# keshaviyengar/gym-ctr-reach

Hardware: AMD Instinct MI355X
Metric: env-steps/sec at 65 536 parallel 3-tube envs; tip-pos L2 vs CPU ref (higher is better)
Workload: dtype f64; 1 GPU; configs[2]: 65536 envs/GPU, 3-tube torsionally-compliant CTR, scipy-RK45 (rtol 1e-3, atol 1e-6) fp64, system 0, n_substeps 10, tol 0.020, max 150 steps, auto-reset; obs_dtype=float32, integrator=rk45_scipy, model=compliant, envs_per_gpu=65536, global_envs=65536, parallelism=env-shard x1, launch=one HIP graph per refill period (2 steps + the refill), replayed

## Files before the change

gym-ctr-reach_amd/csrc/ctr_kernels.hip:

```cpp
#include <hip/hip_runtime.h>
#include <stdint.h>
#include <stdio.h>
#include <string.h>

#include <algorithm>

#include "ctr_device.hpp"
#include "ctr_reach_amd.h"

using namespace ctr;

namespace {

constexpr int BLOCK = 256;

thread_local char g_err[512] = "";

int fail(int code, const char *msg)
{
    snprintf(g_err, sizeof g_err, "%s", msg);
    return code;
}

int hip_check(const char *what)
// ... 462 lines not shown
    #pragma unroll
    for (int i = 27; i < 32; ++i) d[i] = 0u;
    uint4 *v = reinterpret_cast<uint4 *>(sl);
    #pragma unroll
    for (int k = 0; k < 8; ++k) v[k] = make_uint4(d[4 * k], d[4 * k + 1], d[4 * k + 2], d[4 * k + 3]);
}

template <bool ALL = false>
__device__ __forceinline__ void pool_prefetch(const KCfg &kc, const ctr_batch_t &b, int64_t e, int32_t autoreset,
                                              PoolPre &pp, int32_t t, uint32_t epoch)
{
    const int P = b.pool_depth;
    if (!autoreset || P <= 0 || (!ALL && t + 1 < kc.c.max_steps)) return;
    const uint32_t r = epoch + 1;
    pool_load(b.pool + ((int64_t)(r % (uint32_t)P) * b.n + e), pp);
}

struct StepFlags {
    bool miss = false;
    bool pooled = false;
    uint32_t pooled_r = 0;
};

__device__ __forceinline__ void step_finish(const KCfg &kc, const ctr_batch_t &b, const ctr_step_out_t &o, int64_t e,
                                            int s, float q[6], double ag[3], const FkStats &st, int32_t autoreset,
                                            StepFlags &fl, const ctr_her_t *her, const float *action,
                                            PoolPre &lp, int32_t t_prev, uint32_t epoch, const double dg_prev[3],
                                            float4 &grow)
{
    const int32_t t = t_prev + 1;
    double dg[3];
    #pragma unroll
    for (int i = 0; i < 3; ++i) dg[i] = dg_prev[i];
    const double dx = ag[0] - dg[0], dy = ag[1] - dg[1], dz = ag[2] - dg[2];
    const double d = sqrt(dx * dx + dy * dy + dz * dz);
    const double tol = kc.c.tol;
    const float reward = (d > tol) ? -1.0f : 0.0f;
    const bool done = (reward == 0.0f) || (t >= kc.c.max_steps);
    const bool multi = kc.c.n_systems > 1;
    const bool f64 = kc.c.obs_f64 != 0;
    double obs[14];
    obs_lane(q, dg, ag, tol, s, multi, kc.c.egocentric != 0, obs);
    o.reward[e] = reward;
    o.done[e] = done ? 1 : 0;
    o.success[e] = (d < tol) ? 1 : 0;
    o.error[e] = (float)d;
    uint32_t stat = st.status;
    if (o.nfev) o.nfev[e] = st.nfev;
    if (o.packed || o.gather) {
        const float fl = (float)((done ? 1 : 0) | ((d < tol) ? 2 : 0) | ((reward < 0.0f) ? 4 : 0));
        const float4 row = make_float4((float)ag[0], (float)ag[1], (float)ag[2], fl);
        if (o.packed) *reinterpret_cast<float4 *>(o.packed + 4 * e) = row;
        grow = row;
    }
    if (her) {
        float obf[14];
        obs_to_f32(obs, obf);
        her_record_lane(*her, e, action, reward, done, obf, ag, tol);
    }
    int32_t t_out = t;
    if (autoreset && done) {
        if (o.terminal_obs) write_obs(o.terminal_obs, e, obs, multi, f64);
        if (o.terminal_achieved)
            #pragma unroll
            for (int i = 0; i < 3; ++i) o.terminal_achieved[3 * e + i] = ag[i];
        const uint32_t r = epoch + 1;
        const int P = b.pool_depth;
        if (P > 0 && !lp.loaded) pool_load(b.pool + ((int64_t)(r % (uint32_t)P) * b.n + e), lp);
        if (P > 0 && lp.pr == r) {
            const int s2 = clamp_sys(lp.sys, kc.c.n_systems);
            #pragma unroll
            for (int i = 0; i < 6; ++i) q[i] = lp.q0[i];
            #pragma unroll
            for (int i = 0; i < 3; ++i) {
                dg[i] = lp.dg[i];
                ag[i] = lp.ag[i];
            }
            if (b.desired_joints)
                #pragma unroll
                for (int i = 0; i < 6; ++i) b.desired_joints[6 * e + i] = lp.qd[i];
            if (b.starting_joints)
                #pragma unroll
                for (int i = 0; i < 6; ++i) b.starting_joints[6 * e + i] = q[i];
            if (b.starting_position)
                #pragma unroll
                for (int i = 0; i < 3; ++i) b.starting_position[3 * e + i] = ag[i];
            #pragma unroll
            for (int i = 0; i < 3; ++i) b.desired_goal[3 * e + i] = dg[i];
            b.system[e] = s2;
            b.epoch[e] = r;
            stat |= lp.stat;
            obs_lane(q, dg, ag, kc.c.tol, s2, multi, kc.c.egocentric != 0, obs);
            if (her) {
                float obf[14];
                obs_to_f32(obs, obf);
                her_reopen(*her, e, r, obf, ag, dg);
            }
            fl.pooled = true;
            fl.pooled_r = r;
            t_out = 0;
        } else if (autoreset == CTR_AUTORESET_POOLED) {
            stat |= CTR_STATUS_POOL_MISS;
        } else {
            fl.miss = true;
        }
    }
    b.t[e] = t_out;
    #pragma unroll
    for (int i = 0; i < 6; ++i) b.joints[6 * e + i] = q[i];
    #pragma unroll
    for (int i = 0; i < 3; ++i) b.achieved_goal[3 * e + i] = ag[i];
    write_obs(o.obs, e, obs, multi, f64);
    if (o.status) o.status[e] = stat;
}

template <int G = SEG_GROUP>
__device__ __forceinline__ void step_finish_group(const KCfg &kc, const ctr_batch_t &b, const ctr_step_out_t &o,
                                                  int64_t e, int j, bool in, int s, const float q[6], double ag[3],
                                                  const FkStats &st, int32_t autoreset, StepFlags &fl,
                                                  PoolPre &pp, float4 &grow)
{
    const int lead = (int)(threadIdx.x & 63) & ~(G - 1);
    #pragma unroll
    for (int i = 0; i < 3; ++i) ag[i] = __shfl(ag[i], lead);
    if (!in || j > 1) return;
    const int32_t t = b.t[e] + 1;
    double dg[3];
    #pragma unroll
    for (int i = 0; i < 3; ++i) dg[i] = b.desired_goal[3 * e + i];
    const double dx = ag[0] - dg[0], dy = ag[1] - dg[1], dz = ag[2] - dg[2];
    const double d = sqrt(dx * dx + dy * dy + dz * dz);
    const double tol = kc.c.tol;
    const float reward = (d > tol) ? -1.0f : 0.0f;
    const bool done = (reward == 0.0f) || (t >= kc.c.max_steps);
    const bool multi = kc.c.n_systems > 1;
    const bool f64 = kc.c.obs_f64 != 0;
// ... 50 lines not shown
            #pragma unroll
            for (int i = 0; i < 6; ++i) b.desired_joints[6 * e + i] = pp.qd[i];
        if (b.starting_joints)
            #pragma unroll
            for (int i = 0; i < 6; ++i) b.starting_joints[6 * e + i] = pp.q0[i];
        if (b.starting_position)
            #pragma unroll
            for (int i = 0; i < 3; ++i) b.starting_position[3 * e + i] = pp.ag[i];
        #pragma unroll
        for (int i = 0; i < 3; ++i) { b.desired_goal[3 * e + i] = pp.dg[i]; b.achieved_goal[3 * e + i] = pp.ag[i]; }
        #pragma unroll
        for (int i = 0; i < 6; ++i) b.joints[6 * e + i] = pp.q0[i];
        b.system[e] = so;
        b.epoch[e] = r;
        b.t[e] = 0;
        write_obs(o.obs, e, obs, multi, f64);
        fl.pooled = true;
        fl.pooled_r = r;
    }
}

__device__ __forceinline__ void step_epilogue(const ctr_batch_t &b, const ctr_step_out_t &o, int32_t autoreset,
                                              const StepFlags &fl, int64_t e, bool live, const ctr_gather_push_t *gp,
                                              bool slot_free0, float4 grow)
{
    if (autoreset) {
        if (autoreset == CTR_AUTORESET_POOLED) {
            if (blockIdx.x == 0 && threadIdx.x == 0) b.work[(b.work_parity & 1) ^ 1] = 0;
        } else {
            const int32_t one[1] = {(int32_t)e};
            wave_append(miss_counter(b), miss_items(b), b.n, fl.miss, one, 1);
        }
        if (b.pool_depth > 0) {
            const int32_t two[2] = {(int32_t)e, (int32_t)(fl.pooled_r + (uint32_t)b.pool_depth)};
            wave_append(b.refill, b.refill + 1, b.refill_cap, fl.pooled, two, 2);
        }
    }
    if (gp) {
        if (!slot_free0 && !gather_wait_slot(gp, o.gather_seq)) {
            if ((threadIdx.x & 63) == 0) atomicOr(gp->err, CTR_GATHER_E_RELEASE_TIMEOUT);
            gather_poison_lanes(gp, o.gather_seq);
        }
        if (live) gather_store_row(gp, e, grow);
        gather_rows_performed();
        if (o.gather_wait_prev && blockIdx.x == 0 && threadIdx.x < 64)
            gather_wait_prev_lane(gp, o.gather_seq - 1u);
    }
}

template <int MODE, bool HER>
__device__ __forceinline__ void step_body(const KCfg &kc, const ctr_batch_t &b, const float *__restrict__ actions,
                                          const ctr_step_out_t &o, int32_t autoreset, const HerK &hk)
{
    const ctr_her_t *her = HER ? &hk.h : nullptr;
    constexpr bool GROUP = (MODE & 6) == 6;
    constexpr int G = GROUP ? SEG_GROUP : 1;
    __shared__ SysK s_sys[CTR_MAX_SYSTEMS];
    __shared__ ctr_tube_raw_t s_raw[CTR_MAX_SYSTEMS];
    const int64_t gl = (int64_t)blockIdx.x * BLOCK + threadIdx.x;
    const int64_t e = gl / G;
    const int j = (int)(gl % G);
    const bool in = e < b.n;
    const bool live = in && j == 0;
    StageRegs stg;
    stage_load(kc, stg);
    __builtin_amdgcn_sched_barrier(0);
    const int64_t ec = in ? e : b.n - 1;
    const int s_in = b.system[ec];
    float q_in[6], a_in[6];
    #pragma unroll
    for (int i = 0; i < 6; ++i) { q_in[i] = b.joints[6 * ec + i]; a_in[i] = actions[6 * ec + i]; }
    const int32_t t_in = b.t[ec];
    const uint32_t ep_in = b.epoch[ec];
    double dg_in[3];
    #pragma unroll
    for (int i = 0; i < 3; ++i) dg_in[i] = b.desired_goal[3 * ec + i];
    const ctr_gather_push_t *gp = o.gather;
    const uint32_t rel0 = gp ? gather_release_load(gp, o.gather_seq) : 0u;
    stage_systems<!GROUP>(kc, s_sys, s_raw, &stg);
    const bool slot_free0 = gp ? gather_slot_free(gp, o.gather_seq, rel0) : true;
    __shared__ double s_fin_dg[3][BLOCK];
    __shared__ int32_t s_fin_t[BLOCK];
    __shared__ uint32_t s_fin_ep[BLOCK];
    if constexpr (!GROUP) {
        #pragma unroll
        for (int i = 0; i < 3; ++i) s_fin_dg[i][threadIdx.x] = dg_in[i];
        s_fin_t[threadIdx.x] = t_in;
        s_fin_ep[threadIdx.x] = ep_in;
    }
    if (o.packed && o.packed_seq && blockIdx.x == 0 && threadIdx.x == 0)
        *reinterpret_cast<uint4 *>(o.packed + 4 * b.n) = make_uint4(o.packed_seq, 0u, 0u, 0u);
    if (blockIdx.x == 0) {
        if (o.gather_prev) gather_publish_lane(o.gather_prev, o.gather_prev_seq);
        if (gp) gather_release_lane(gp, o.gather_seq + 1u - (uint32_t)gp->depth);
    }
    StepFlags fl;
    float4 grow = make_float4(0.f, 0.f, 0.f, 0.f);
    if constexpr (GROUP) {
        int s = 0;
        float q[6] = {0.f, 0.f, 0.f, 0.f, 0.f, 0.f};
        PoolPre pp;
        if (in && j == (HER ? 0 : 1)) pool_prefetch<true>(kc, b, e, autoreset, pp, t_in, ep_in);
        if (in) {
            s = clamp_sys(s_in, kc.c.n_systems);
            #pragma unroll
            for (int i = 0; i < 6; ++i) q[i] = q_in[i];
            set_action_substeps(s_sys[s], kc.c.constrain_alpha != 0, kc.c.n_substeps, q, a_in);
        }
        const SysK &sy = in ? episode_sys(kc, s_sys, s_raw, s, b.epoch[e], (uint64_t)(b.env_base + e)) : s_sys[0];
        const double qd[6] = {(double)q[0], (double)q[1], (double)q[2], (double)q[3], (double)q[4], (double)q[5]};
        FkStats st = {0, 0, 0, 0, 0};
        double ag[3];
        if (fk_needs_careful_trig(qd))
            fk_group_rigid4<(MODE & 1) != 0, true>(sy, qd, j, ag, st, (double)kc.c.rk4_steps_per_m);
        else
            fk_group_rigid4<(MODE & 1) != 0, false>(sy, qd, j, ag, st, (double)kc.c.rk4_steps_per_m);
        if constexpr (HER) {
            if (live)
                step_finish(kc, b, o, e, s, q, ag, st, autoreset, fl, her, actions + 6 * e, pp, t_in, ep_in, dg_in, grow);
        } else {
            step_finish_group(kc, b, o, e, j, in, s, q, ag, st, autoreset, fl, pp, grow);
        }
    } else if (live) {
        const int s = clamp_sys(s_in, kc.c.n_systems);
        const SysK &sy = s_sys[s];
        float q[6];
        #pragma unroll
        for (int i = 0; i < 6; ++i) q[i] = q_in[i];
        PoolPre pp;
        pool_prefetch(kc, b, e, autoreset, pp, t_in, ep_in);
        set_action_substeps(sy, kc.c.constrain_alpha != 0, kc.c.n_substeps, q, a_in);
        FkStats st = {0, 0, 0, 0, 0};
        double ag[3];
        fk_dispatch<MODE>(kc, episode_sys(kc, s_sys, s_raw, s, ep_in, (uint64_t)(b.env_base + e)), q, ag, st);
        double dg_f[3];
        #pragma unroll
        for (int i = 0; i < 3; ++i) dg_f[i] = s_fin_dg[i][threadIdx.x];
        step_finish(kc, b, o, e, s, q, ag, st, autoreset, fl, her, actions + 6 * e, pp, s_fin_t[threadIdx.x],
                    s_fin_ep[threadIdx.x], dg_f, grow);
    }
    step_epilogue(b, o, autoreset, fl, e, live, gp, slot_free0, grow);
}

#ifndef CTR_RK4_PAIR
#define CTR_RK4_PAIR 1
#endif
#ifndef CTR_RK45_PAIR
#define CTR_RK45_PAIR 0
#endif
template <int MODE>
constexpr bool pair_mode() { return (CTR_RK4_PAIR && MODE == 2) || (CTR_RK45_PAIR && MODE == 0); }
template <int MODE>
constexpr int step_block() { return pair_mode<MODE>() ? 2 * BLOCK : BLOCK; }
template <int MODE>
constexpr int step_lanes_per_env() { return pair_mode<MODE>() ? 2 : ((MODE & 6) == 6 ? SEG_GROUP : 1); }

__device__ __forceinline__ int pair_work_bucket(const ctr_system_t &sy, const float q[6], double inv_wmax)
{
    const double e2 = fmax(0.0, (double)q[2] + sy.L[2]);
    const double e1 = fmax(e2, (double)q[1] + sy.L[1]);
    const double w = (4.0 * e2 + 3.0 * (e1 - e2)) * inv_wmax;
    return 255 - (int)fmin(fmax(w * 255.0, 0.0), 255.0);
}

// ... 121 lines not shown
            step_finish(kc, b, o, e, s, q, ag, st, autoreset, fl, her, actions + 6 * e, pp, t_in, ep_in, dg_in, grow);
        }
    } else {
        step_finish_group<2>(kc, b, o, e, j, in, s, q, ag, st, autoreset, fl, pp, grow);
    }
    step_epilogue(b, o, autoreset, fl, e, live, gp, slot_free0, grow);
}

template <int MODE>
__global__ __launch_bounds__(step_block<MODE>()) void k_step(KCfg kc, ctr_batch_t b, const float *__restrict__ actions,
                                                                ctr_step_out_t o, int32_t autoreset)
{
    if constexpr (pair_mode<MODE>()) step_body_pair<MODE, false>(kc, b, actions, o, autoreset, HerK{});
    else step_body<MODE, false>(kc, b, actions, o, autoreset, HerK{});
}

template <int MODE>
__global__ __launch_bounds__(step_block<MODE>()) void k_step_her(KCfg kc, ctr_batch_t b,
                                                                    const float *__restrict__ actions,
                                                                    ctr_step_out_t o, int32_t autoreset, HerK hk)
{
    if constexpr (pair_mode<MODE>()) step_body_pair<MODE, true>(kc, b, actions, o, autoreset, hk);
    else step_body<MODE, true>(kc, b, actions, o, autoreset, hk);
}

struct ResetOut {
    float qd[6], q0[6];
    double dg[3], ag[3];
    int sys;
    uint32_t stat;
};

template <int MODE>
struct ResetLanes {
    static constexpr bool GROUP = (MODE & 6) == 6;
    static constexpr int U = GROUP ? 2 * SEG_GROUP : 2;
    static constexpr int PX = GROUP ? SEG_GROUP : 1;
    __device__ static bool odd() { return ((threadIdx.x & 63) / PX) & 1; }
    __device__ static int j() { return GROUP ? (int)(threadIdx.x & (SEG_GROUP - 1)) : 0; }
    __device__ static bool writer() { return odd() && j() == 0; }
};

template <int MODE>
__device__ __forceinline__ ResetOut reset_pair(const KCfg &kc, const SysK *s_sys, const ctr_tube_raw_t *s_raw,
                                               bool active, bool odd,
                                               uint64_t genv, uint32_t r, const float *q_cur, const double *goal,
// ... 646 lines not shown
            CTR_LAUNCH(k_step, kc.mode, dim3(grid_for(lanes)), lane_lds_bytes(kc), s, kc, b, actions, o, autoreset);
    }
    if (int r = hip_check("ctr_step launch")) return r;
    if (autoreset == CTR_AUTORESET_SWEEP) {
        const unsigned g = b.pool_depth > 0 ? std::min(grid_for(reset_lanes(kc) * b.n), 64u)
                                            : grid_for(reset_lanes(kc) * b.n);
        CTR_LAUNCH(k_reset, kc.mode, dim3(g), lane_lds_bytes(kc), s, kc, b, 0, (const uint8_t *)nullptr, (const double *)nullptr,
                   (const int32_t *)nullptr, o.obs, o.status, hk, her_on);
        return hip_check("ctr_step reset launch");
    }
    return 0;
}

}

extern "C" {

int ctr_step(const ctr_env_config_t *cfg, const ctr_batch_t *batch, const float *actions, const ctr_step_out_t *out,
             int32_t autoreset, void *stream)
{
    return step_launch(cfg, batch, actions, out, autoreset, nullptr, stream);
}

int ctr_reset(const ctr_env_config_t *cfg, const ctr_batch_t *batch, const uint8_t *mask, const double *goal,
              const int32_t *system, void *obs, uint32_t *status, void *stream)
{
    if (int r = check_cfg(cfg)) return r;
    if (!batch || !obs) return fail(CTR_EINVAL, "ctr_reset: NULL argument");
    const ctr_batch_t b = *batch;
    if (int r = check_batch(b, "ctr_reset: batch buffer missing")) return r;
    if (b.n == 0) return 0;
    if (b.pool_depth > 0 && !cfg->resample_joints) return fail(CTR_EINVAL, "the reset pool needs resample_joints");
    KCfg kc = make_kcfg(cfg);
    CTR_LAUNCH(k_reset, kc.mode, dim3(grid_for(reset_lanes(kc) * b.n)), lane_lds_bytes(kc), (hipStream_t)stream, kc, b, 1, mask,
               goal, system, obs,
               status, HerK{}, 0);
    return hip_check("ctr_reset launch");
}

int ctr_pool_refill(const ctr_env_config_t *cfg, const ctr_batch_t *batch, void *stream)
{
    if (int r = check_cfg(cfg)) return r;
    if (!batch) return fail(CTR_EINVAL, "ctr_pool_refill: NULL argument");
    const ctr_batch_t b = *batch;
    if (int r = check_batch(b, "ctr_pool_refill: batch buffer missing")) return r;
    if (b.n == 0 || b.pool_depth == 0) return 0;
// ... 54 lines not shown
```

gym-ctr-reach_amd/ctr_reach_amd/_abi.py:

```python
import ctypes
import os

HERE = os.path.dirname(os.path.abspath(__file__))
LIB_PATH = os.environ.get("CTR_REACH_AMD_LIB") or os.path.join(HERE, "lib", "libctr_reach_amd.so")

CTR_ABI_VERSION = 15
CTR_IPC_HANDLE_BYTES = 64
CTR_GATHER_MAX_RANKS = 16
CTR_MAX_SYSTEMS = 8
CTR_POOL_MAX = 192
CTR_HER_SCAN_TILE = 1024
CTR_INTEGRATOR_RK45_SCIPY = 0
CTR_INTEGRATOR_RK4 = 1
CTR_MODEL_COMPLIANT = 0
CTR_MODEL_RIGID = 1
CTR_STATUS_STEP_UNDERFLOW = 1
CTR_STATUS_SAMPLER_STUCK = 2
CTR_STATUS_NAN = 4
CTR_STATUS_TOO_LONG = 8
CTR_STATUS_POOL_MISS = 16
AUTORESET_OFF = 0
AUTORESET_SWEEP = 1
AUTORESET_POOLED = 2
CTR_HER_FUTURE = 0
CTR_HER_FINAL = 1
CTR_HER_EPISODE = 2

_d3 = ctypes.c_double * 3
_P = ctypes.c_void_p


class CtrSystem(ctypes.Structure):
    _fields_ = [("L", _d3), ("Lc", _d3), ("EI", _d3), ("GJ", _d3), ("Ux", _d3), ("Uy", _d3)]
# ... 72 lines not shown
class CtrStepOut(ctypes.Structure):
    _fields_ = [
        ("obs", _P),
        ("reward", _P),
        ("done", _P),
        ("success", _P),
        ("error", _P),
        ("terminal_obs", _P),
        ("terminal_achieved", _P),
        ("status", _P),
        ("nfev", _P),
        ("packed", _P),
        ("packed_seq", ctypes.c_uint32),
        ("packed_pad", ctypes.c_uint32),
        ("gather", _P),
        ("gather_prev", _P),
        ("gather_prev_seq", ctypes.c_uint32),
        ("gather_seq", ctypes.c_uint32),
        ("gather_wait_prev", ctypes.c_int32),
        ("gather_pad", ctypes.c_int32),
    ]


class CtrGatherPush(ctypes.Structure):
    _fields_ = [("src", _P), ("n", ctypes.c_int64), ("world", ctypes.c_int32), ("pad", ctypes.c_int32),
                ("dst", _P * CTR_GATHER_MAX_RANKS), ("seqw", _P * CTR_GATHER_MAX_RANKS), ("ticket", _P),
                ("relw", _P * CTR_GATHER_MAX_RANKS), ("rel", _P), ("wait_seqw", _P), ("err", _P),
                ("depth", ctypes.c_int32), ("wait_us", ctypes.c_uint32),
                ("poisonw", _P * CTR_GATHER_MAX_RANKS), ("poison", _P)]


CTR_GATHER_E_WAIT_TIMEOUT = 1
CTR_GATHER_E_OVERWRITTEN = 2
CTR_GATHER_E_RELEASE_TIMEOUT = 4
CTR_GATHER_E_PREV_TIMEOUT = 8


class CtrCopy(ctypes.Structure):
    _fields_ = [("dst", _P), ("src", _P), ("bytes", ctypes.c_int64), ("stream", ctypes.c_int32),
                ("pad", ctypes.c_int32)]


class CtrHer(ctypes.Structure):
    _fields_ = [
        ("obs_dim", ctypes.c_int32),
        ("t_max", ctypes.c_int32),
# ... 4 lines not shown
        ("slots", ctypes.c_int32),
        ("pad", ctypes.c_int32),
        ("seed", ctypes.c_uint64),
        ("state", _P),
        ("step", _P),
        ("dg", _P),
        ("tol", _P),
        ("len", _P),
        ("epoch", _P),
        ("cur_t", _P),
        ("cur_epoch", _P),
        ("cdf", _P),
    ]


class CtrHerBatch(ctypes.Structure):
    _fields_ = [("obs", _P), ("action", _P), ("reward", _P), ("next_obs", _P), ("done", _P), ("index", _P)]


EXPORTED = ("ctr_abi_version", "ctr_last_error", "ctr_fk", "ctr_set_action", "ctr_step", "ctr_reset",
            "ctr_pool_refill", "ctr_compute_reward", "ctr_domain_params", "ctr_fk_tables", "ctr_jacobian", "ctr_fk_shape",
            "ctr_her_open", "ctr_her_record", "ctr_her_sample", "ctr_step_her", "ctr_pool_requeue",
            "ctr_ipc_get_handle", "ctr_ipc_open", "ctr_ipc_close", "ctr_seqw_alloc", "ctr_seqw_free", "ctr_copy_list",
            "ctr_gather_wait", "ctr_gather_push", "ctr_gather_publish", "ctr_refill_carry_bytes")

_lib = None


class CtrError(RuntimeError):
    pass


def load(path=None):
    global _lib
    if _lib is not None:
        return _lib
    path = path or LIB_PATH
    if not os.path.exists(path):
        raise CtrError("libctr_reach_amd.so not built (%s); run __graft_entry__.build()" % path)
    L = ctypes.CDLL(path)
    i64, i32 = ctypes.c_int64, ctypes.c_int32
    L.ctr_abi_version.restype = ctypes.c_int
    L.ctr_last_error.restype = ctypes.c_char_p
    L.ctr_fk.argtypes = [_P, _P, i64, ctypes.POINTER(CtrEnvConfig), _P, _P, _P, _P]
    L.ctr_set_action.argtypes = [ctypes.POINTER(CtrEnvConfig), _P, _P, _P, i64, _P]
    L.ctr_step.argtypes = [ctypes.POINTER(CtrEnvConfig), ctypes.POINTER(CtrBatch), _P,
                           ctypes.POINTER(CtrStepOut), i32, _P]
# ... 8 lines not shown
    L.ctr_her_open.argtypes = [ctypes.POINTER(CtrHer), ctypes.POINTER(CtrBatch), _P, _P, _P]
    L.ctr_her_record.argtypes = [ctypes.POINTER(CtrHer), ctypes.POINTER(CtrBatch), _P, ctypes.POINTER(CtrStepOut),
                                 ctypes.c_double, _P]
    L.ctr_her_sample.argtypes = [ctypes.POINTER(CtrHer), i64, ctypes.c_uint64, ctypes.c_uint64,
                                 ctypes.POINTER(CtrHerBatch), _P]
    L.ctr_step_her.argtypes = [ctypes.POINTER(CtrEnvConfig), ctypes.POINTER(CtrBatch), _P,
                               ctypes.POINTER(CtrStepOut), i32, ctypes.POINTER(CtrHer), _P]
    try:
        L.ctr_ipc_get_handle.argtypes = [_P, _P]
        L.ctr_ipc_open.argtypes = [_P, ctypes.POINTER(_P)]
        L.ctr_ipc_close.argtypes = [_P]
        L.ctr_seqw_alloc.argtypes = [i64, ctypes.POINTER(_P)]
        L.ctr_seqw_free.argtypes = [_P]
        L.ctr_copy_list.argtypes = [ctypes.POINTER(CtrCopy), i32, ctypes.POINTER(_P), i32, _P, ctypes.POINTER(_P)]
        L.ctr_gather_wait.argtypes = [_P, i32, ctypes.c_uint32, ctypes.c_uint32, _P, _P]
        L.ctr_gather_push.argtypes = [ctypes.POINTER(CtrGatherPush), ctypes.c_uint32, i32, _P]
        L.ctr_gather_publish.argtypes = [_P, ctypes.c_uint32, _P]
    except AttributeError:
        if L.ctr_abi_version() == CTR_ABI_VERSION:
            raise
    for fn in EXPORTED[2:]:
        if hasattr(L, fn):
            getattr(L, fn).restype = ctypes.c_int
    if hasattr(L, "ctr_refill_carry_bytes"):
        L.ctr_refill_carry_bytes.argtypes = [i64]
        L.ctr_refill_carry_bytes.restype = i64
    allowed = {CTR_ABI_VERSION, int(os.environ.get("CTR_REACH_AMD_ALLOW_ABI", CTR_ABI_VERSION))}
    if L.ctr_abi_version() not in allowed:
        raise CtrError("ABI version mismatch: library %d, binding %d" % (L.ctr_abi_version(), CTR_ABI_VERSION))
    _lib = L
    return L


def check(rc, what):
    if rc != 0:
        msg = _lib.ctr_last_error().decode() if _lib is not None else ""
        raise CtrError("%s failed (rc=%d): %s" % (what, rc, msg))


def ptr(t):
    if t is None:
        return None
    return ctypes.c_void_p(t.data_ptr())


def stream_ptr(stream=None, device_index=None):
# ... 7 lines not shown
```

gym-ctr-reach_amd/ctr_reach_amd/vec_env.py:

```python
import numpy as np

from . import _abi
from . import distributed as D
from .goal_tolerance import GoalTolerance
from .spaces import Box, Dict
from .systems import default_kwargs, make_config, solver_codes, tubes_from_params

NUM_TUBES = 3
EXT_TOL = 1e-3
ZERO_TOL = 1e-4
RK4_REFILL_BUDGET = 32


def _torch():
    import torch
    return torch


def _current_stream(stream, device):
    import torch
    return stream if stream is not None else torch.cuda.current_stream(device)


def joint_spaces(systems, constrain_alpha):
# ... 17 lines not shown
    rep = Box(low=np.array(rep_low), high=np.array(rep_high), dtype="float32")
    if len(systems) == 1:
        lo = np.concatenate((rep.low, np.array([-0.2, -0.2, -0.2, goal_tolerance.final_tol])))
        hi = np.concatenate((rep.high, np.array([0.2, 0.2, 0.2, goal_tolerance.init_tol])))
    else:
        lo = np.concatenate((rep.low, np.array([-0.2, -0.2, -0.2, goal_tolerance.final_tol, 0])))
        hi = np.concatenate((rep.high, np.array([0.2, 0.2, 0.2, goal_tolerance.init_tol, len(systems) - 1])))
    return Dict(dict(
        desired_goal=Box(low=np.array([-0.1, -0.1, 0]), high=np.array([0.1, 0.1, 0.2]), dtype="float32"),
        achieved_goal=Box(low=np.array([-0.1, -0.1, 0]), high=np.array([0.1, 0.1, 0.2]), dtype="float32"),
        observation=Box(low=lo, high=hi, dtype="float32")))


def action_space(extension_action_limit, rotation_action_limit):
    b = np.full(NUM_TUBES, extension_action_limit)
    a = np.full(NUM_TUBES, np.deg2rad(rotation_action_limit))
    return Box(low=np.concatenate((-b, -a)), high=np.concatenate((b, a)), dtype="float32")


class CtrReachVecEnv(object):

    def __init__(self, num_envs, device="cuda", seed=0, env_base=0, autoreset=True, record_info=True,
                 pool_depth=None, refill_interval=64, integrator="rk45_scipy", rk4_steps_per_m=100,
                 model="compliant", pack_outputs=False, obs_dtype="float32", refill_budget=None, **kwargs):
        torch = _torch()
        kw = default_kwargs()
        kw.update(kwargs)
        if kw.get("length_based_sample"):
            raise NotImplementedError("length_based_sample: the reference branch is broken "
                                      "(reads the nonexistent self.system_parameters, ctr_reach_env.py:88)")
        assert kw["joint_representation"] in ("egocentric", "proprioceptive")
        self.kwargs = kw
        self.integrator, self.rk4_steps_per_m, self.model = integrator, int(rk4_steps_per_m), model
        solver = solver_codes(integrator, rk4_steps_per_m, model)
        self.lib = _abi.load()
        self.num_envs = int(num_envs)
        self.device = torch.device(device)
        self.env_base = int(env_base)
        self.autoreset = bool(autoreset)
        all_systems = tubes_from_params(kw["ctr_systems_parameters"])
        self.select_systems = list(kw["select_systems"])
        self.ctr_system_parameters = [all_systems[s] for s in self.select_systems]
        self.n_systems = len(self.ctr_system_parameters)
        self.goal_tolerance = GoalTolerance(kw["goal_tolerance_parameters"])
        self.max_steps_per_episode = kw["max_steps_per_episode"]
        self.n_substeps = kw["n_substeps"]
        self.constrain_alpha = kw["constrain_alpha"]
# ... 25 lines not shown
        self.t = torch.zeros(n, dtype=i32, device=dev)
        self.system = torch.zeros(n, dtype=i32, device=dev)
        self.epoch = torch.zeros(n, dtype=i32, device=dev)
        self.work = torch.zeros(n + 2, dtype=i32, device=dev)
        self.desired_joints = torch.zeros((n, 6), dtype=f32, device=dev) if record_info else None
        self.starting_joints = torch.zeros((n, 6), dtype=f32, device=dev) if record_info else None
        self.starting_position = torch.zeros((n, 3), dtype=f64, device=dev) if record_info else None
        self.obs = torch.zeros((n, self.obs_dim), dtype=self.obs_dtype, device=dev)
        self.reward = torch.zeros(n, dtype=f32, device=dev)
        self.done = torch.zeros(n, dtype=torch.uint8, device=dev)
        self.success = torch.zeros(n, dtype=torch.uint8, device=dev)
        self.error = torch.zeros(n, dtype=f32, device=dev)
        self.terminal_obs = torch.zeros((n, self.obs_dim), dtype=self.obs_dtype, device=dev)
        self.terminal_achieved = torch.zeros((n, 3), dtype=f64, device=dev)
        self.status = torch.zeros(n, dtype=i32, device=dev)
        self.nfev = None
        self.packed_bufs = [torch.zeros((n + 1, D.PACK_WIDTH), dtype=f32, device=dev) for _ in range(2)] if pack_outputs else None
        self._packed_k = 0
        self.packed_seq = 0
        self._push_gather = None
        self.gather_seq = 0
        self.refills = 0
        self.sweeps = 0
        R = max(1, int(refill_interval))
        resumable = not (integrator == "rk4" and model == "rigid")
        if refill_budget is None:
            refill_budget = (6 if integrator == "rk45_scipy" else RK4_REFILL_BUDGET) if resumable else 0
        if refill_budget and not resumable:
            raise ValueError("refill_budget is not available for the rigid model's fixed-step RK4 (its FKs run as "
                             "segment maps)")
        if pool_depth is None:
            want = 2 * R + 24 if refill_budget else R
            pool_depth = max(8, min(64, want)) if (self.autoreset and self.resample_joints) else 0
        if pool_depth and not self.resample_joints:
            raise ValueError("the reset pool needs resample_joints=True")
        self.pool_depth = int(pool_depth)
        self.refill_interval = R
        self.refill_budget = int(refill_budget) if (self.pool_depth > 2 * R) else 0
        self.refill_lead = R
        self._steps_since_refill = 0
        self._pool_full = False
        P = self.pool_depth
        if P:
            self.pool = torch.zeros((P, n, _abi.POOL_SLOT_DWORDS), dtype=i32, device=dev)
            if self.pool.data_ptr() % 128:
                raise RuntimeError("reset pool not 128-B aligned")
# ... 158 lines not shown
            else:
                mode = _abi.AUTORESET_SWEEP
                self.sweeps += 1
        if her is not None and her.fused:
            rc = self.lib.ctr_step_her(self.cfg, self._batch, _abi.ptr(actions), self._out, mode, her._h, sp)
        else:
            rc = self.lib.ctr_step(self.cfg, self._batch, _abi.ptr(actions), self._out, mode, sp)
        if fused:
            o.gather = o.gather_prev = None
            o.gather_wait_prev = 0
            if rc == 0:
                g.stepped(self.gather_seq)
        if rc:
            _abi.check(rc, "ctr_step")
        if her is not None and not her.fused:
            her._record(actions, stream)
        if self.autoreset:
            self._batch.work_parity ^= 1
        if self.pool_depth:
            self._steps_since_refill += 1
            if self._steps_since_refill >= self.refill_interval:
                self.refill_pool(stream)

    def capture_steps(self, actions, stream=None):
        return StepGraph(self, actions, stream)

    def compute_reward(self, achieved_goal, desired_goal, info=None):
        torch = _torch()
        tol = float(self.goal_tolerance.get_tol())
        if isinstance(achieved_goal, torch.Tensor):
            assert achieved_goal.shape == desired_goal.shape
            shape = achieved_goal.shape[:-1]
            ag = achieved_goal.to(self.device, torch.float64).reshape(-1, 3).contiguous()
            dg = desired_goal.to(self.device, torch.float64).reshape(-1, 3).contiguous()
            out = torch.empty(ag.shape[0], dtype=torch.float32, device=self.device)
            rc = self.lib.ctr_compute_reward(_abi.ptr(ag), _abi.ptr(dg), ag.shape[0], tol, _abi.ptr(out),
                                             _abi.stream_ptr())
            _abi.check(rc, "ctr_compute_reward")
            return out.reshape(shape)
        achieved_goal = np.asarray(achieved_goal)
        desired_goal = np.asarray(desired_goal)
        assert achieved_goal.shape == desired_goal.shape
        d = np.linalg.norm(achieved_goal - desired_goal, axis=-1)
        return -(d > tol).astype(np.float64)

    def forward_kinematics(self, joints, system=None, stream=None, return_stats=False, tables=None):
# ... 152 lines not shown
    def close(self):
        pass


class StepGraph(object):

    def __init__(self, env, actions, stream=None):
        torch = _torch()
        k = len(actions)
        if env._her is not None or env._push_gather is not None:
            raise RuntimeError("capture_steps: not with the HER feed or the push gather")
        if env.autoreset and env.pool_depth:
            if k % env.refill_interval or env._steps_since_refill != 0 or not env._pool_full:
                raise RuntimeError("capture_steps: start right after a refill with a full pool and capture a "
                                   "multiple of refill_interval (%d) steps" % env.refill_interval)
        elif env.autoreset:
            raise RuntimeError("capture_steps: auto-reset needs the reset pool")
        if k % 2:
            raise RuntimeError("capture_steps: an even number of steps (buffer parities)")
        self.env, self.steps = env, k
        self.actions = [a for a in actions]
        self.stream = stream if stream is not None else torch.cuda.Stream(device=env.device)
        self.stream.wait_stream(torch.cuda.current_stream(env.device))
        refills, sweeps, seq = env.refills, env.sweeps, env.packed_seq
        self.graph = torch.cuda.CUDAGraph()
        with torch.cuda.graph(self.graph, stream=self.stream):
            for a in self.actions:
                env.step_raw(a, self.stream)
        self.refills_per_replay = env.refills - refills
        env.refills, env.sweeps, env.packed_seq = refills, sweeps, seq
        assert env._steps_since_refill == 0 or not env.pool_depth

    def replay(self):
        self.graph.replay()
        self.env.refills += self.refills_per_replay
        if self.env.packed_bufs is not None:
            self.env.packed_seq += self.steps
```

include/ctr_reach_amd.h:

```cpp
#ifndef CTR_REACH_AMD_H
#define CTR_REACH_AMD_H

#include <stdint.h>

#ifdef __cplusplus
extern "C" {
#endif

#define CTR_ABI_VERSION 15
#define CTR_MAX_SYSTEMS 8
#define CTR_POOL_MAX 192
#define CTR_EINVAL (-1)
#define CTR_EHIP (-2)

#define CTR_STATUS_STEP_UNDERFLOW 1u
#define CTR_STATUS_SAMPLER_STUCK  2u
#define CTR_STATUS_NAN            4u
#define CTR_STATUS_TOO_LONG       8u
#define CTR_STATUS_POOL_MISS     16u

#define CTR_AUTORESET_OFF    0
#define CTR_AUTORESET_SWEEP  1
#define CTR_AUTORESET_POOLED 2

typedef struct ctr_system_t {
    double L[3];
    double Lc[3];
    double EI[3];
    double GJ[3];
    double Ux[3];
    double Uy[3];
} ctr_system_t;
// ... 141 lines not shown

int ctr_abi_version(void);
const char *ctr_last_error(void);

int ctr_fk(const float *joints, const int32_t *sys_idx, int64_t n, const ctr_env_config_t *cfg,
           double *tip, uint32_t *stats, uint32_t *status, void *stream);

int ctr_fk_tables(const float *joints, const ctr_system_t *tables, int64_t n, const ctr_env_config_t *cfg,
                  double *tip, uint32_t *stats, uint32_t *status, void *stream);

int ctr_fk_shape(const float *joints, const int32_t *sys_idx, const ctr_system_t *tables, int64_t n,
                 const ctr_env_config_t *cfg, int32_t cap, double *tip, double *r, double *s, int32_t *npts,
                 uint32_t *status, void *stream);

int ctr_jacobian(const double *joints, const int32_t *sys_idx, int64_t n, const ctr_env_config_t *cfg, double eps,
                 double *tip, double *jac, uint32_t *status, void *stream);

int ctr_set_action(const ctr_env_config_t *cfg, float *joints, const int32_t *sys_idx,
                   const float *actions, int64_t n, void *stream);

int ctr_step(const ctr_env_config_t *cfg, const ctr_batch_t *batch, const float *actions,
             const ctr_step_out_t *out, int32_t autoreset, void *stream);

int ctr_reset(const ctr_env_config_t *cfg, const ctr_batch_t *batch, const uint8_t *mask,
              const double *goal, const int32_t *system, void *obs, uint32_t *status, void *stream);

int ctr_pool_refill(const ctr_env_config_t *cfg, const ctr_batch_t *batch, void *stream);

int64_t ctr_refill_carry_bytes(int64_t carry_cap);

int ctr_pool_requeue(const ctr_env_config_t *cfg, const ctr_batch_t *batch, void *stream);

int ctr_domain_params(const ctr_env_config_t *cfg, const ctr_batch_t *batch, ctr_system_t *sys_out,
                      ctr_tube_raw_t *raw_out, void *stream);

#define CTR_IPC_HANDLE_BYTES 64
#define CTR_GATHER_MAX_RANKS 16
#define CTR_GATHER_E_WAIT_TIMEOUT    1u
#define CTR_GATHER_E_OVERWRITTEN     2u
#define CTR_GATHER_E_RELEASE_TIMEOUT 4u
#define CTR_GATHER_E_PREV_TIMEOUT    8u

struct ctr_gather_push_t {
    const void *src;
    int64_t     n;
    int32_t     world;
// ... 47 lines not shown
```

Measured before the change: 548.8 million env-steps/s.

## Fuse multiple env steps per refill period into one persistent step_many kernel

Adds a k_step_many kernel that runs up to 64 consecutive env steps in one launch. Per-env state (joints, system, t, epoch, goal) stays in registers between steps, and the next action is prefetched into LDS. The graph capture uses it by default when the pool holds every reset for the period. This removes per-step launch overhead and the repeated global reloads of env state and shared system tables. In exchange, the kernel's register pressure may rise, and the RK45 step count varies per lane, so divergence now accumulates across steps inside one wave.

```diff
diff --git a/gym-ctr-reach_amd/csrc/ctr_kernels.hip b/gym-ctr-reach_amd/csrc/ctr_kernels.hip
--- a/gym-ctr-reach_amd/csrc/ctr_kernels.hip
+++ b/gym-ctr-reach_amd/csrc/ctr_kernels.hip
@@ -508,11 +508,18 @@
     uint32_t pooled_r = 0;
 };
 
+struct StepCarry {
+    int s;
+    int32_t t;
+    uint32_t ep;
+    double dg[3];
+};
+
 __device__ __forceinline__ void step_finish(const KCfg &kc, const ctr_batch_t &b, const ctr_step_out_t &o, int64_t e,
                                             int s, float q[6], double ag[3], const FkStats &st, int32_t autoreset,
                                             StepFlags &fl, const ctr_her_t *her, const float *action,
                                             PoolPre &lp, int32_t t_prev, uint32_t epoch, const double dg_prev[3],
-                                            float4 &grow)
+                                            float4 &grow, StepCarry *nx = nullptr)
 {
     const int32_t t = t_prev + 1;
     double dg[3];
@@ -545,6 +552,7 @@
         her_record_lane(*her, e, action, reward, done, obf, ag, tol);
     }
     int32_t t_out = t;
+    if (nx) { nx->s = s; nx->ep = epoch; }
     if (autoreset && done) {
         if (o.terminal_obs) write_obs(o.terminal_obs, e, obs, multi, f64);
         if (o.terminal_achieved)
@@ -585,6 +593,7 @@
             fl.pooled = true;
             fl.pooled_r = r;
             t_out = 0;
+            if (nx) { nx->s = s2; nx->ep = r; }
         } else if (autoreset == CTR_AUTORESET_POOLED) {
             stat |= CTR_STATUS_POOL_MISS;
         } else {
@@ -598,6 +607,11 @@
     for (int i = 0; i < 3; ++i) b.achieved_goal[3 * e + i] = ag[i];
     write_obs(o.obs, e, obs, multi, f64);
     if (o.status) o.status[e] = stat;
+    if (nx) {
+        nx->t = t_out;
+        #pragma unroll
+        for (int i = 0; i < 3; ++i) nx->dg[i] = dg[i];
+    }
 }
 
 template <int G = SEG_GROUP>
@@ -694,11 +708,11 @@
 
 __device__ __forceinline__ void step_epilogue(const ctr_batch_t &b, const ctr_step_out_t &o, int32_t autoreset,
                                               const StepFlags &fl, int64_t e, bool live, const ctr_gather_push_t *gp,
-                                              bool slot_free0, float4 grow)
+                                              bool slot_free0, float4 grow, bool zero_miss = true)
 {
     if (autoreset) {
         if (autoreset == CTR_AUTORESET_POOLED) {
-            if (blockIdx.x == 0 && threadIdx.x == 0) b.work[(b.work_parity & 1) ^ 1] = 0;
+            if (zero_miss && blockIdx.x == 0 && threadIdx.x == 0) b.work[(b.work_parity & 1) ^ 1] = 0;
         } else {
             const int32_t one[1] = {(int32_t)e};
             wave_append(miss_counter(b), miss_items(b), b.n, fl.miss, one, 1);
@@ -718,6 +732,126 @@
         if (o.gather_wait_prev && blockIdx.x == 0 && threadIdx.x < 64)
             gather_wait_prev_lane(gp, o.gather_seq - 1u);
     }
+}
+
+struct StepRows {
+    int s;
+    float q[6], a[6];
+    int32_t t;
+    uint32_t ep;
+    double dg[3];
+};
+
+__device__ __forceinline__ void step_rows_load(const ctr_batch_t &b, const float *__restrict__ actions, int64_t ec,
+                                               StepRows &r)
+{
+    r.s = b.system[ec];
+    #pragma unroll
+    for (int i = 0; i < 6; ++i) { r.q[i] = b.joints[6 * ec + i]; r.a[i] = actions[6 * ec + i]; }
+    r.t = b.t[ec];
+    r.ep = b.epoch[ec];
+    #pragma unroll
+    for (int i = 0; i < 3; ++i) r.dg[i] = b.desired_goal[3 * ec + i];
+}
+
+__device__ __forceinline__ float (*next_action_lds())[BLOCK]
+{
+    __shared__ float s_next_a[6][BLOCK];
+    return s_next_a;
+}
+
+template <int MODE, bool HER, bool MANY>
+__device__ __forceinline__ void step_one(const KCfg &kc, const ctr_batch_t &b, const float *__restrict__ actions,
+                                         const ctr_step_out_t &o, int32_t autoreset, const ctr_her_t *her,
+                                         const SysK *s_sys, const ctr_tube_raw_t *s_raw, int64_t e, int j, bool in,
+                                         bool live, StepRows &r, const ctr_gather_push_t *gp, bool slot_free0,
+                                         const float *__restrict__ next_actions)
+{
+    constexpr bool GROUP = (MODE & 6) == 6;
+    static_assert(!MANY || (!GROUP && !HER), "k_step_many: one env per lane, no HER");
+    __shared__ double s_fin_dg[3][BLOCK];
+    __shared__ int32_t s_fin_t[BLOCK];
+    __shared__ uint32_t s_fin_ep[BLOCK];
+    if constexpr (!GROUP) {
+        #pragma unroll
+        for (int i = 0; i < 3; ++i) s_fin_dg[i][threadIdx.x] = r.dg[i];
+        s_fin_t[threadIdx.x] = r.t;
+        s_fin_ep[threadIdx.x] = r.ep;
+    }
+    if constexpr (!MANY) {
+        if (o.packed && o.packed_seq && blockIdx.x == 0 && threadIdx.x == 0)
+            *reinterpret_cast<uint4 *>(o.packed + 4 * b.n) = make_uint4(o.packed_seq, 0u, 0u, 0u);
+        if (blockIdx.x == 0) {
+            if (o.gather_prev) gather_publish_lane(o.gather_prev, o.gather_prev_seq);
+            if (gp) gather_release_lane(gp, o.gather_seq + 1u - (uint32_t)gp->depth);
+        }
+    }
+    StepFlags fl;
+    float4 grow = make_float4(0.f, 0.f, 0.f, 0.f);
+    if constexpr (GROUP) {
+        int s = 0;
+        float q[6] = {0.f, 0.f, 0.f, 0.f, 0.f, 0.f};
+        PoolPre pp;
+        if (in && j == (HER ? 0 : 1)) pool_prefetch<true>(kc, b, e, autoreset, pp, r.t, r.ep);
+        if (in) {
+            s = clamp_sys(r.s, kc.c.n_systems);
+            #pragma unroll
+            for (int i = 0; i < 6; ++i) q[i] = r.q[i];
+            set_action_substeps(s_sys[s], kc.c.constrain_alpha != 0, kc.c.n_substeps, q, r.a);
+        }
+        const SysK &sy = in ? episode_sys(kc, s_sys, s_raw, s, b.epoch[e], (uint64_t)(b.env_base + e)) : s_sys[0];
+        const double qd[6] = {(double)q[0], (double)q[1], (double)q[2], (double)q[3], (double)q[4], (double)q[5]};
+        FkStats st = {0, 0, 0, 0, 0};
+        double ag[3];
+        if (fk_needs_careful_trig(qd))
+            fk_group_rigid4<(MODE & 1) != 0, true>(sy, qd, j, ag, st, (double)kc.c.rk4_steps_per_m);
+        else
+            fk_group_rigid4<(MODE & 1) != 0, false>(sy, qd, j, ag, st, (double)kc.c.rk4_steps_per_m);
+        if constexpr (HER) {
+            if (live)
+                step_finish(kc, b, o, e, s, q, ag, st, autoreset, fl, her, actions + 6 * e, pp, r.t, r.ep, r.dg, grow);
+        } else {
+            step_finish_group(kc, b, o, e, j, in, s, q, ag, st, autoreset, fl, pp, grow);
+        }
+    } else if (live) {
+        const int s = clamp_sys(r.s, kc.c.n_systems);
+        const SysK &sy = s_sys[s];
+        float q[6];
+        #pragma unroll
+        for (int i = 0; i < 6; ++i) q[i] = r.q[i];
+        float a_nx[6] = {0.f, 0.f, 0.f, 0.f, 0.f, 0.f};
+        if constexpr (MANY) {
+            if (next_actions)
+                #pragma unroll
+                for (int i = 0; i < 6; ++i) a_nx[i] = next_actions[6 * e + i];
+        }
+        PoolPre pp;
+        pool_prefetch(kc, b, e, autoreset, pp, r.t, r.ep);
+        set_action_substeps(sy, kc.c.constrain_alpha != 0, kc.c.n_substeps, q, r.a);
+        if constexpr (MANY) {
+            #pragma unroll
+            for (int i = 0; i < 6; ++i) next_action_lds()[i][threadIdx.x] = a_nx[i];
+        }
+        FkStats st = {0, 0, 0, 0, 0};
+        double ag[3];
+        fk_dispatch<MODE>(kc, episode_sys(kc, s_sys, s_raw, s, r.ep, (uint64_t)(b.env_base + e)), q, ag, st);
+        double dg_f[3];
+        #pragma unroll
+        for (int i = 0; i < 3; ++i) dg_f[i] = s_fin_dg[i][threadIdx.x];
+        StepCarry nx;
+        step_finish(kc, b, o, e, s, q, ag, st, autoreset, fl, her, MANY ? nullptr : actions + 6 * e, pp,
+                    s_fin_t[threadIdx.x], s_fin_ep[threadIdx.x], dg_f, grow, MANY ? &nx : nullptr);
+        if constexpr (MANY) {
+            r.s = nx.s;
+            r.t = nx.t;
+            r.ep = nx.ep;
+            #pragma unroll
+            for (int i = 0; i < 3; ++i) r.dg[i] = nx.dg[i];
+            #pragma unroll
+            for (int i = 0; i < 6; ++i) { r.q[i] = q[i]; r.a[i] = next_action_lds()[i][threadIdx.x]; }
+        }
+    }
+    step_epilogue(b, o, autoreset, fl, e, live, gp, slot_free0, grow, !MANY);
 }
 
 template <int MODE, bool HER>
@@ -737,81 +871,40 @@
     StageRegs stg;
     stage_load(kc, stg);
     __builtin_amdgcn_sched_barrier(0);
-    const int64_t ec = in ? e : b.n - 1;
-    const int s_in = b.system[ec];
-    float q_in[6], a_in[6];
-    #pragma unroll
-    for (int i = 0; i < 6; ++i) { q_in[i] = b.joints[6 * ec + i]; a_in[i] = actions[6 * ec + i]; }
-    const int32_t t_in = b.t[ec];
-    const uint32_t ep_in = b.epoch[ec];
-    double dg_in[3];
-    #pragma unroll
-    for (int i = 0; i < 3; ++i) dg_in[i] = b.desired_goal[3 * ec + i];
+    StepRows r;
+    step_rows_load(b, actions, in ? e : b.n - 1, r);
     const ctr_gather_push_t *gp = o.gather;
     const uint32_t rel0 = gp ? gather_release_load(gp, o.gather_seq) : 0u;
     stage_systems<!GROUP>(kc, s_sys, s_raw, &stg);
     const bool slot_free0 = gp ? gather_slot_free(gp, o.gather_seq, rel0) : true;
-    __shared__ double s_fin_dg[3][BLOCK];
-    __shared__ int32_t s_fin_t[BLOCK];
-    __shared__ uint32_t s_fin_ep[BLOCK];
-    if constexpr (!GROUP) {
-        #pragma unroll
-        for (int i = 0; i < 3; ++i) s_fin_dg[i][threadIdx.x] = dg_in[i];
-        s_fin_t[threadIdx.x] = t_in;
-        s_fin_ep[threadIdx.x] = ep_in;
-    }
-    if (o.packed && o.packed_seq && blockIdx.x == 0 && threadIdx.x == 0)
-        *reinterpret_cast<uint4 *>(o.packed + 4 * b.n) = make_uint4(o.packed_seq, 0u, 0u, 0u);
-    if (blockIdx.x == 0) {
-        if (o.gather_prev) gather_publish_lane(o.gather_prev, o.gather_prev_seq);
-        if (gp) gather_release_lane(gp, o.gather_seq + 1u - (uint32_t)gp->depth);
-    }
-    StepFlags fl;
-    float4 grow = make_float4(0.f, 0.f, 0.f, 0.f);
-    if constexpr (GROUP) {
-        int s = 0;
-        float q[6] = {0.f, 0.f, 0.f, 0.f, 0.f, 0.f};
-        PoolPre pp;
-        if (in && j == (HER ? 0 : 1)) pool_prefetch<true>(kc, b, e, autoreset, pp, t_in, ep_in);
-        if (in) {
-            s = clamp_sys(s_in, kc.c.n_systems);
-            #pragma unroll
-            for (int i = 0; i < 6; ++i) q[i] = q_in[i];
-            set_action_substeps(s_sys[s], kc.c.constrain_alpha != 0, kc.c.n_substeps, q, a_in);
-        }
-        const SysK &sy = in ? episode_sys(kc, s_sys, s_raw, s, b.epoch[e], (uint64_t)(b.env_base + e)) : s_sys[0];
-        const double qd[6] = {(double)q[0], (double)q[1], (double)q[2], (double)q[3], (double)q[4], (double)q[5]};
-        FkStats st = {0, 0, 0, 0, 0};
-        double ag[3];
-        if (fk_needs_careful_trig(qd))
-            fk_group_rigid4<(MODE & 1) != 0, true>(sy, qd, j, ag, st, (double)kc.c.rk4_steps_per_m);
-        else
-            fk_group_rigid4<(MODE & 1) != 0, false>(sy, qd, j, ag, st, (double)kc.c.rk4_steps_per_m);
-        if constexpr (HER) {
-            if (live)
-                step_finish(kc, b, o, e, s, q, ag, st, autoreset, fl, her, actions + 6 * e, pp, t_in, ep_in, dg_in, grow);
-        } else {
-            step_finish_group(kc, b, o, e, j, in, s, q, ag, st, autoreset, fl, pp, grow);
-        }
-    } else if (live) {
-        const int s = clamp_sys(s_in, kc.c.n_systems);
-        const SysK &sy = s_sys[s];
-        float q[6];
-        #pragma unroll
-        for (int i = 0; i < 6; ++i) q[i] = q_in[i];
-        PoolPre pp;
-        pool_prefetch(kc, b, e, autoreset, pp, t_in, ep_in);
-        set_action_substeps(sy, kc.c.constrain_alpha != 0, kc.c.n_substeps, q, a_in);
-        FkStats st = {0, 0, 0, 0, 0};
-        double ag[3];
-        fk_dispatch<MODE>(kc, episode_sys(kc, s_sys, s_raw, s, ep_in, (uint64_t)(b.env_base + e)), q, ag, st);
-        double dg_f[3];
-        #pragma unroll
-        for (int i = 0; i < 3; ++i) dg_f[i] = s_fin_dg[i][threadIdx.x];
-        step_finish(kc, b, o, e, s, q, ag, st, autoreset, fl, her, actions + 6 * e, pp, s_fin_t[threadIdx.x],
-                    s_fin_ep[threadIdx.x], dg_f, grow);
-    }
-    step_epilogue(b, o, autoreset, fl, e, live, gp, slot_free0, grow);
+    step_one<MODE, HER, false>(kc, b, actions, o, autoreset, her, s_sys, s_raw, e, j, in, live, r, gp, slot_free0,
+                               nullptr);
+}
+
+template <int MODE>
+__device__ __forceinline__ void step_body_many(const KCfg &kc, const ctr_batch_t &b, const ctr_action_seq_t &seq,
+                                               int32_t k, const ctr_step_out_t &o, int32_t autoreset)
+{
+    __shared__ SysK s_sys[CTR_MAX_SYSTEMS];
+    __shared__ ctr_tube_raw_t s_raw[CTR_MAX_SYSTEMS];
+    const int64_t e = (int64_t)blockIdx.x * BLOCK + threadIdx.x;
+    const bool live = e < b.n;
+    StageRegs stg;
+    stage_load(kc, stg);
+    __builtin_amdgcn_sched_barrier(0);
+    StepRows r;
+    step_rows_load(b, seq.a[0], live ? e : b.n - 1, r);
+    stage_systems<true>(kc, s_sys, s_raw, &stg);
+    if (autoreset == CTR_AUTORESET_POOLED && blockIdx.x == 0 && threadIdx.x == 0) {
+        b.work[(b.work_parity & 1) ^ 1] = 0;
+        if (k > 1) b.work[b.work_parity & 1] = 0;
+    }
+    #pragma unroll 1
+    for (int32_t i = 0; i < k; ++i) {
+        const float *nxt = i + 1 < k ? seq.a[i + 1] : nullptr;
+        step_one<MODE, false, true>(kc, b, nullptr, o, autoreset, nullptr, s_sys, s_raw, e, 0, live, live, r, nullptr,
+                                    true, nxt);
+    }
 }
 
 #ifndef CTR_RK4_PAIR
@@ -979,6 +1072,13 @@
 {
     if constexpr (pair_mode<MODE>()) step_body_pair<MODE, true>(kc, b, actions, o, autoreset, hk);
     else step_body<MODE, true>(kc, b, actions, o, autoreset, hk);
+}
+
+template <int MODE>
+__global__ __launch_bounds__(BLOCK) void k_step_many(KCfg kc, ctr_batch_t b, ctr_action_seq_t seq, int32_t k,
+                                                     ctr_step_out_t o, int32_t autoreset)
+{
+    if constexpr (!pair_mode<MODE>() && (MODE & 6) != 6) step_body_many<MODE>(kc, b, seq, k, o, autoreset);
 }
 
 struct ResetOut {
@@ -1671,6 +1771,50 @@
     return step_launch(cfg, batch, actions, out, autoreset, nullptr, stream);
 }
 
+int ctr_step_many(const ctr_env_config_t *cfg, const ctr_batch_t *batch, const ctr_action_seq_t *actions, int32_t k,
+                  const ctr_step_out_t *out, int32_t autoreset, void *stream)
+{
+    if (int r = check_cfg(cfg)) return r;
+    if (!batch || !out || !actions) return fail(CTR_EINVAL, "ctr_step_many: NULL argument");
+    if (k < 1 || k > CTR_STEP_MANY_MAX) return fail(CTR_EINVAL, "ctr_step_many: k must be in 1..CTR_STEP_MANY_MAX (64)");
+    for (int32_t i = 0; i < k; ++i)
+        if (!actions->a[i]) return fail(CTR_EINVAL, "ctr_step_many: NULL action buffer among a[0..k-1]");
+    const ctr_batch_t b = *batch;
+    const ctr_step_out_t o = *out;
+    if (int r = check_batch(b, "ctr_step_many: batch buffer missing")) return r;
+    if (autoreset != CTR_AUTORESET_OFF && autoreset != CTR_AUTORESET_POOLED)
+        return fail(CTR_EINVAL, "ctr_step_many: autoreset must be CTR_AUTORESET_OFF or CTR_AUTORESET_POOLED (a miss sweep "
+                                "is a launch between two steps)");
+    if (o.packed || o.gather || o.gather_prev)
+        return fail(CTR_EINVAL, "ctr_step_many: not with packed rows or the push gather (out->packed, gather, gather_prev)");
+    const KCfg kc = make_kcfg(cfg);
+    if (pair_mode<2>() && kc.mode == 2)
+        return fail(CTR_EINVAL, "ctr_step_many: not for the lane-pair step (compliant model, fixed-step RK4)");
+    if ((kc.mode & 6) == 6)
+        return fail(CTR_EINVAL, "ctr_step_many: not for the 8-lane group step (rigid model, fixed-step RK4)");
+    if (pair_mode<0>() && kc.mode == 0) return fail(CTR_EINVAL, "ctr_step_many: not for the lane-pair step");
+    if (b.n == 0) return 0;
+    if (!o.obs || !o.reward || !o.done || !o.success || !o.error) return fail(CTR_EINVAL, "ctr_step_many: output missing");
+    if (autoreset && !b.work) return fail(CTR_EINVAL, "ctr_step_many: autoreset needs batch->work");
+    if (autoreset == CTR_AUTORESET_POOLED && b.pool_depth <= 0)
+        return fail(CTR_EINVAL, "ctr_step_many: CTR_AUTORESET_POOLED needs a reset pool");
+    if (b.pool_depth > 0 && !cfg->resample_joints) return fail(CTR_EINVAL, "the reset pool needs resample_joints");
+    ctr_action_seq_t seq;
+    for (int32_t i = 0; i < CTR_STEP_MANY_MAX; ++i) seq.a[i] = i < k ? actions->a[i] : nullptr;
+    const dim3 g(grid_for(b.n)), blk(BLOCK);
+    const size_t shm = lane_lds_bytes(kc);
+    hipStream_t s = (hipStream_t)stream;
+    switch (kc.mode) {
+    case 0: hipLaunchKernelGGL(k_step_many<0>, g, blk, shm, s, kc, b, seq, k, o, autoreset); break;
+    case 1: hipLaunchKernelGGL(k_step_many<1>, g, blk, shm, s, kc, b, seq, k, o, autoreset); break;
+    case 2: hipLaunchKernelGGL(k_step_many<2>, g, blk, shm, s, kc, b, seq, k, o, autoreset); break;
+    case 3: hipLaunchKernelGGL(k_step_many<3>, g, blk, shm, s, kc, b, seq, k, o, autoreset); break;
+    case 4: hipLaunchKernelGGL(k_step_many<4>, g, blk, shm, s, kc, b, seq, k, o, autoreset); break;
+    default: hipLaunchKernelGGL(k_step_many<5>, g, blk, shm, s, kc, b, seq, k, o, autoreset); break;
+    }
+    return hip_check("ctr_step_many launch");
+}
+
 int ctr_reset(const ctr_env_config_t *cfg, const ctr_batch_t *batch, const uint8_t *mask, const double *goal,
               const int32_t *system, void *obs, uint32_t *status, void *stream)
 {
diff --git a/gym-ctr-reach_amd/ctr_reach_amd/_abi.py b/gym-ctr-reach_amd/ctr_reach_amd/_abi.py
--- a/gym-ctr-reach_amd/ctr_reach_amd/_abi.py
+++ b/gym-ctr-reach_amd/ctr_reach_amd/_abi.py
@@ -4,11 +4,12 @@
 HERE = os.path.dirname(os.path.abspath(__file__))
 LIB_PATH = os.environ.get("CTR_REACH_AMD_LIB") or os.path.join(HERE, "lib", "libctr_reach_amd.so")
 
-CTR_ABI_VERSION = 15
+CTR_ABI_VERSION = 16
 CTR_IPC_HANDLE_BYTES = 64
 CTR_GATHER_MAX_RANKS = 16
 CTR_MAX_SYSTEMS = 8
 CTR_POOL_MAX = 192
+CTR_STEP_MANY_MAX = 64
 CTR_HER_SCAN_TILE = 1024
 CTR_INTEGRATOR_RK45_SCIPY = 0
 CTR_INTEGRATOR_RK4 = 1
@@ -127,6 +128,10 @@
     ]
 
 
+class CtrActionSeq(ctypes.Structure):
+    _fields_ = [("a", _P * CTR_STEP_MANY_MAX)]
+
+
 class CtrGatherPush(ctypes.Structure):
     _fields_ = [("src", _P), ("n", ctypes.c_int64), ("world", ctypes.c_int32), ("pad", ctypes.c_int32),
                 ("dst", _P * CTR_GATHER_MAX_RANKS), ("seqw", _P * CTR_GATHER_MAX_RANKS), ("ticket", _P),
@@ -177,7 +182,7 @@
             "ctr_pool_refill", "ctr_compute_reward", "ctr_domain_params", "ctr_fk_tables", "ctr_jacobian", "ctr_fk_shape",
             "ctr_her_open", "ctr_her_record", "ctr_her_sample", "ctr_step_her", "ctr_pool_requeue",
             "ctr_ipc_get_handle", "ctr_ipc_open", "ctr_ipc_close", "ctr_seqw_alloc", "ctr_seqw_free", "ctr_copy_list",
-            "ctr_gather_wait", "ctr_gather_push", "ctr_gather_publish", "ctr_refill_carry_bytes")
+            "ctr_gather_wait", "ctr_gather_push", "ctr_gather_publish", "ctr_refill_carry_bytes", "ctr_step_many")
 
 _lib = None
 
@@ -232,6 +237,9 @@
     for fn in EXPORTED[2:]:
         if hasattr(L, fn):
             getattr(L, fn).restype = ctypes.c_int
+    if hasattr(L, "ctr_step_many"):
+        L.ctr_step_many.argtypes = [ctypes.POINTER(CtrEnvConfig), ctypes.POINTER(CtrBatch), ctypes.POINTER(CtrActionSeq),
+                                    i32, ctypes.POINTER(CtrStepOut), i32, _P]
     if hasattr(L, "ctr_refill_carry_bytes"):
         L.ctr_refill_carry_bytes.argtypes = [i64]
         L.ctr_refill_carry_bytes.restype = i64
diff --git a/gym-ctr-reach_amd/ctr_reach_amd/vec_env.py b/gym-ctr-reach_amd/ctr_reach_amd/vec_env.py
--- a/gym-ctr-reach_amd/ctr_reach_amd/vec_env.py
+++ b/gym-ctr-reach_amd/ctr_reach_amd/vec_env.py
@@ -1,3 +1,5 @@
+import os
+
 import numpy as np
 
 from . import _abi
@@ -63,7 +65,8 @@
 
     def __init__(self, num_envs, device="cuda", seed=0, env_base=0, autoreset=True, record_info=True,
                  pool_depth=None, refill_interval=64, integrator="rk45_scipy", rk4_steps_per_m=100,
-                 model="compliant", pack_outputs=False, obs_dtype="float32", refill_budget=None, **kwargs):
+                 model="compliant", pack_outputs=False, obs_dtype="float32", refill_budget=None, fused_period=True,
+                 **kwargs):
         torch = _torch()
         kw = default_kwargs()
         kw.update(kwargs)
@@ -135,6 +138,8 @@
         self.gather_seq = 0
         self.refills = 0
         self.sweeps = 0
+        self.fused_period = bool(fused_period) and os.environ.get("CTR_FUSED_PERIOD", "1") != "0"
+        self.fused_launches = 0
         R = max(1, int(refill_interval))
         resumable = not (integrator == "rk4" and model == "rigid")
         if refill_budget is None:
@@ -339,6 +344,58 @@
             if self._steps_since_refill >= self.refill_interval:
                 self.refill_pool(stream)
 
+    def step_many_ineligible(self):
+        if self._her is not None:
+            return "not with the HER feed"
+        if self._push_gather is not None or self.packed_bufs is not None:
+            return "not with packed outputs or the push gather"
+        if self.integrator == "rk4":
+            if self.model == "rigid":
+                return "not for the rigid model's fixed-step RK4 (8-lane group step)"
+            uy = any(self.cfg.systems[s].Uy[i] != 0.0 for s in range(self.n_systems) for i in range(3))
+            if not uy:
+                return "not for the compliant model's fixed-step RK4 (lane-pair step)"
+        if self.autoreset and not (self.pool_depth and self._pool_full):
+            return "auto-reset needs the reset pool, full (every reset of the steps precomputed)"
+        return None
+
+    def step_many(self, actions, stream=None):
+        torch = _torch()
+        why = self.step_many_ineligible()
+        if why:
+            raise RuntimeError("step_many: " + why)
+        actions = list(actions)
+        for a in actions:
+            if (a.dtype != torch.float32 or a.device != self.device or not a.is_contiguous()
+                    or a.shape != (self.num_envs, 6)):
+                raise ValueError("step_many: actions must be contiguous float32 [%d, 6] tensors on %s"
+                                 % (self.num_envs, self.device))
+        sp = _abi.stream_ptr(stream, self.device.index)
+        i = 0
+        while i < len(actions):
+            k = min(len(actions) - i, _abi.CTR_STEP_MANY_MAX)
+            if self.pool_depth:
+                k = min(k, self.refill_interval - self._steps_since_refill)
+            mode = _abi.AUTORESET_OFF
+            if self.autoreset:
+                k = min(k, self._pooled_steps() - self._steps_since_refill)
+                if k < 1 or not self._pool_full:
+                    raise RuntimeError("step_many: the next step's resets are not all in the pool")
+                mode = _abi.AUTORESET_POOLED
+            seq = _abi.CtrActionSeq()
+            for j in range(k):
+                seq.a[j] = actions[i + j].data_ptr()
+            rc = self.lib.ctr_step_many(self.cfg, self._batch, seq, k, self._out, mode, sp)
+            _abi.check(rc, "ctr_step_many")
+            self.fused_launches += 1
+            if self.autoreset and k % 2:
+                self._batch.work_parity ^= 1
+            if self.pool_depth:
+                self._steps_since_refill += k
+                if self._steps_since_refill >= self.refill_interval:
+                    self.refill_pool(stream)
+            i += k
+
     def capture_steps(self, actions, stream=None):
         return StepGraph(self, actions, stream)
 
@@ -537,17 +594,23 @@
         self.actions = [a for a in actions]
         self.stream = stream if stream is not None else torch.cuda.Stream(device=env.device)
         self.stream.wait_stream(torch.cuda.current_stream(env.device))
-        refills, sweeps, seq = env.refills, env.sweeps, env.packed_seq
+        refills, sweeps, seq, fused = env.refills, env.sweeps, env.packed_seq, env.fused_launches
+        self.fused = env.fused_period and env.step_many_ineligible() is None
         self.graph = torch.cuda.CUDAGraph()
         with torch.cuda.graph(self.graph, stream=self.stream):
-            for a in self.actions:
-                env.step_raw(a, self.stream)
+            if self.fused:
+                env.step_many(self.actions, self.stream)
+            else:
+                for a in self.actions:
+                    env.step_raw(a, self.stream)
         self.refills_per_replay = env.refills - refills
-        env.refills, env.sweeps, env.packed_seq = refills, sweeps, seq
+        self.fused_per_replay = env.fused_launches - fused
+        env.refills, env.sweeps, env.packed_seq, env.fused_launches = refills, sweeps, seq, fused
         assert env._steps_since_refill == 0 or not env.pool_depth
 
     def replay(self):
         self.graph.replay()
         self.env.refills += self.refills_per_replay
+        self.env.fused_launches += self.fused_per_replay
         if self.env.packed_bufs is not None:
             self.env.packed_seq += self.steps
diff --git a/include/ctr_reach_amd.h b/include/ctr_reach_amd.h
--- a/include/ctr_reach_amd.h
+++ b/include/ctr_reach_amd.h
@@ -7,7 +7,7 @@
 extern "C" {
 #endif
 
-#define CTR_ABI_VERSION 15
+#define CTR_ABI_VERSION 16
 #define CTR_MAX_SYSTEMS 8
 #define CTR_POOL_MAX 192
 #define CTR_EINVAL (-1)
@@ -195,6 +195,13 @@
 int ctr_step(const ctr_env_config_t *cfg, const ctr_batch_t *batch, const float *actions,
              const ctr_step_out_t *out, int32_t autoreset, void *stream);
 
+#define CTR_STEP_MANY_MAX 64
+typedef struct ctr_action_seq_t {
+    const float *a[CTR_STEP_MANY_MAX];
+} ctr_action_seq_t;
+int ctr_step_many(const ctr_env_config_t *cfg, const ctr_batch_t *batch, const ctr_action_seq_t *actions,
+                  int32_t k, const ctr_step_out_t *out, int32_t autoreset, void *stream);
+
 int ctr_reset(const ctr_env_config_t *cfg, const ctr_batch_t *batch, const uint8_t *mask,
               const double *goal, const int32_t *system, void *obs, uint32_t *status, void *stream);
 
```

Result: faster. 554.8 million env-steps/s, median of 6 (+1.1%).
